# Thraix/VoxelRayTracer

Hardware: AMD Instinct MI355X
Metric: Mrays/sec + achieved HBM GB/s, 1920x1080 @ 128^3 voxels, 4 bounces (higher is better)
Workload: dtype f32

## Files before the change

### voxelraytracer_amd/csrc/vrt_cert.h

```cpp
#ifndef VRT_CERT_H
#define VRT_CERT_H

#include "vrt_walk.h"

namespace vrt {


enum : int { CERT_MISS = 0, CERT_HIT = 1, CERT_UNSURE = 2 };
constexpr int kCertRun = 3;
constexpr float kCertMargin = 1.0f / 64.0f;
constexpr int kCertMaxIter = 1024;
constexpr float kCertMaxOrigin = 4e-3f;

struct CertResult {
  int res;
  uint32_t byte;
  int axis;
  int cx, cy, cz;
  float u;
  float eu;
  float us;
  CERT_DIAG_ONLY(int iters;)
};

__device__ __forceinline__ uint32_t cell_texel(const Ctx& c, int i, int j, int k, uint32_t obase) {
  return load_u16_at(c.vox, mad24(mad24(uint32_t(k), c.p, uint32_t(j)), c.p, uint32_t(i)), obase);
}
__device__ __forceinline__ uint32_t path_texel(const Ctx& c, int i, int j, int k, uint32_t obase) {
  const uint32_t n = uint32_t(c.n);
  if (uint32_t(i) >= n || uint32_t(j) >= n || uint32_t(k) >= n) return 0u;
  return cell_texel(c, i, j, k, obase);
}
constexpr uint32_t kTexOutside = 0x10000u;
__device__ __forceinline__ uint32_t cross_texel(const Ctx& c, int i, int j, int k, uint32_t obase) {
  const bool outside = max(max(uint32_t(i), uint32_t(j)), uint32_t(k)) >= uint32_t(c.n);
  const uint32_t idx = mad24(mad24(uint32_t(k), c.p, uint32_t(j)), c.p, uint32_t(i));
  uint32_t t = load_u16_at(c.vox, outside ? 0u : idx, obase);
  t = outside ? kTexOutside : t;
  asm volatile("" : "+v"(t));
  return t;
}
__device__ __forceinline__ bool cross_outside(uint32_t tex) { return tex >= kTexOutside; }
__device__ __forceinline__ uint32_t start_texel(const Ctx& c, int i, int j, int k, uint32_t obase) {
  const bool outside = max(max(uint32_t(i), uint32_t(j)), uint32_t(k)) >= uint32_t(c.n);
  const uint32_t idx = mad24(mad24(uint32_t(k), c.p, uint32_t(j)), c.p, uint32_t(i));
  const uint32_t t = load_u16_at(c.vox, outside ? 0u : idx, obase);
  return outside ? 0u : t;
}
__device__ __forceinline__ uint32_t alt_byte(const Ctx& c, int i, int j, int k, uint32_t obase) {
  const uint32_t n = uint32_t(c.n);
  if (uint32_t(i) > n || uint32_t(j) > n || uint32_t(k) > n) return 0u;
  return cell_texel(c, i, j, k, obase) & kVoxMask;
}
template <bool SHADOW>
__device__ __forceinline__ bool cert_event(uint32_t b, uint32_t medium) {
  return SHADOW ? (b & ~2u) != 0u : b != medium;
}

struct CertStartK {
  f3 Ps, fl1;
  int mx, my, mz;
  float b0, U2;
};
typedef const __attribute__((address_space(4))) KArgs LateKArgs;
__device__ __forceinline__ LateKArgs* late_kargs() {
  LateKArgs* ka = (LateKArgs*)__builtin_amdgcn_kernarg_segment_ptr();
  asm volatile("" : "+s"(ka));
  return ka;
}

template <bool SHADOW, bool LEAN = false, bool ED = true>
__device__ __forceinline__ CertResult cert_walk(const Ctx& c, const f3 P, const f3 D, const f3 rcp, const float U,
                                int cx, int cy, int cz, const float e0, const f3 ed,
                                const float len0b, const uint32_t medium, const uint32_t tex0 = ~0u,
                                const CertStartK* __restrict__ st0 = nullptr,
                                LateKArgs* sk = nullptr) {
  CertResult r;
  r.res = CERT_UNSURE;
  r.byte = 0u;
  r.axis = 0;
  r.cx = r.cy = r.cz = 0;
  r.u = 0.0f;
  r.eu = 0.0f;
  r.us = 0.0f;
  const bool ksun = LEAN && sk != nullptr;
  const bool kst = LEAN && st0 != nullptr;
  const int sx = ksun ? sk->sun_step[0] : (D.x > 0.0f ? 1 : -1), sy = ksun ? sk->sun_step[1] : (D.y > 0.0f ? 1 : -1),
            sz = ksun ? sk->sun_step[2] : (D.z > 0.0f ? 1 : -1);
  const int ux = ksun ? (sk->sun_step[0] > 0 ? 1 : 0) : (D.x > 0.0f ? 1 : 0), uy = ksun ? (sk->sun_step[1] > 0 ? 1 : 0) : (D.y > 0.0f ? 1 : 0),
            uz = ksun ? (sk->sun_step[2] > 0 ? 1 : 0) : (D.z > 0.0f ? 1 : 0);
  const f3 ar = mk(__builtin_fabsf(rcp.x), __builtin_fabsf(rcp.y), __builtin_fabsf(rcp.z));
  const float l1 = ksun ? sk->sun_l1 : __builtin_fabsf(D.x) + __builtin_fabsf(D.y) + __builtin_fabsf(D.z);
  const uint32_t obase =
      ksun ? sk->sun_obase : ((D.x < 0.0f ? 1u : 0u) | (D.y < 0.0f ? 2u : 0u) | (D.z < 0.0f ? 4u : 0u)) * c.ostride;
  constexpr float k24 = 2.0f * 0x1p-24f;
  const float q2 = ksun ? sk->sun_q2 : 0.5f * k24 * l1;
  const float lin = 6.0f + l1 * (len0b + 1.0f),
              con = (18.0f * 1.0000020f) * __builtin_amdgcn_rcpf(l1) + 3.0f * (len0b + 1.0f);
  const float a1 = k24 * (lin + 2.0f), b1 = ksun ? sk->sun_b1 : k24 * l1,
              b0 = kst ? st0->b0 : (ksun ? sk->walk_b0 : k24 * (3.0f * c.fn + 11.0f));
  const float c0 = k24 * (con + 2.0f * len0b) + 4e-5f + e0;
  const float g2 = ksun ? sk->sun_g2 : 2.0f * q2, g1 = 2.0f * k24 * lin, g0 = 2.0f * k24 * con + 1e-4f + e0;
  const f3 Ps = kst    ? st0->Ps
                : ksun ? mk(__uint_as_float(__float_as_uint(P.x) ^ sk->sun_neg[0]), __uint_as_float(__float_as_uint(P.y) ^ sk->sun_neg[1]),
                            __uint_as_float(__float_as_uint(P.z) ^ sk->sun_neg[2]))
                       : mk(ux ? P.x : -P.x, uy ? P.y : -P.y, uz ? P.z : -P.z);
  const f3 Da = mk(__builtin_fabsf(D.x), __builtin_fabsf(D.y), __builtin_fabsf(D.z));
  const int mx = kst ? st0->mx : ux - 1, my = kst ? st0->my : uy - 1, mz = kst ? st0->mz : uz - 1;
  f3 sig = kst ? mk((st0->fl1.x - Ps.x) * ar.x, (st0->fl1.y - Ps.y) * ar.y, (st0->fl1.z - Ps.z) * ar.z)
               : mk((float(cx + ux) - P.x) * rcp.x, (float(cy + uy) - P.y) * rcp.y, (float(cz + uz) - P.z) * rcp.z);
  uint32_t tex = (tex0 != ~0u ? tex0
                              : (LEAN ? start_texel(c, cx + sx, cy + sy, cz + sz, obase)
                                      : path_texel(c, cx + sx, cy + sy, cz + sz, obase))) +
                 (1u << kDistShift);
  CTRACE(c, 100 + int(SHADOW), cx, cy, cz, P.x, P.y, P.z, U);
  CTRACE(c, 101, D.x, D.y, D.z, e0, ed.x, ed.y, ed.z);
  CERT_DIAG_ONLY(r.iters = 0;)
  if (LEAN && PHASE_STOP(SHADOW ? 4 : 2)) {
    r.u = ((sig.x + sig.y) + (sig.z + q2)) + ((a1 + b1) + (b0 + c0)) + ((g2 + g1) + (g0 + Ps.x)) +
          ((Ps.y + Ps.z) + (Da.x + Da.y)) + ((Da.z + ar.x) + (ar.y + ar.z)) + U;
    r.cx = int(tex + obase) + mx + my + mz;
    return r;
  }
  int st = CERT_UNSURE;
  for (int guard = 0; guard < kCertMaxIter; ++guard) {
    CERT_DIAG_ONLY(r.iters = guard + 1;)
    const float s1 = __builtin_fminf(sig.x, __builtin_fminf(sig.y, sig.z));
    const float uu = gmax(s1, 0.0f);
    const float A = __builtin_fmaf(__builtin_fmaf(q2, uu, a1), uu, c0);
    const float B = __builtin_fmaf(b1, uu, b0);
    auto gam_of = [&](float arb, float edb) {
      const float g = __builtin_fmaf(B, arb, A);
      return ED ? g + edb : g;
    };
    const uint32_t G = tex >> kDistShift;
    bool jumped = false;
    if (SHADOW || medium == 0u) {
      const float fg1 = float(G) - (1.0f + kCertMargin);
      const float fb = fg1 - B;
      const float jx = __builtin_fmaf(fb, ar.x, sig.x), jy = __builtin_fmaf(fb, ar.y, sig.y),
                  jz = __builtin_fmaf(fb, ar.z, sig.z);
      const float jm = ED ? __builtin_fminf(jx - ed.x, __builtin_fminf(jy - ed.y, jz - ed.z))
                          : __builtin_fminf(jx, __builtin_fminf(jy, jz));
      const float uj = __builtin_fminf(jm - A, kst ? st0->U2 : U + 2.0f);
      CTRACE(c, 102, G, s1, uj, gam_of(ar.x, ed.x), gam_of(ar.y, ed.y), gam_of(ar.z, ed.z), 0);
      if (uj > s1) {
        const float fx = __builtin_floorf(__builtin_fmaf(uj, Da.x, Ps.x)),
                    fy = __builtin_floorf(__builtin_fmaf(uj, Da.y, Ps.y)),
                    fz = __builtin_floorf(__builtin_fmaf(uj, Da.z, Ps.z));
        cx = int(fx) ^ mx;
        cy = int(fy) ^ my;
        cz = int(fz) ^ mz;
        if constexpr (LEAN)
          sig = mk(((fx + 1.0f) - Ps.x) * ar.x, ((fy + 1.0f) - Ps.y) * ar.y, ((fz + 1.0f) - Ps.z) * ar.z);
        else
          sig = mk((float(cx + ux) - P.x) * rcp.x, (float(cy + uy) - P.y) * rcp.y, (float(cz + uz) - P.z) * rcp.z);
        tex = LEAN ? cell_texel(c, cx, cy, cz, obase) : path_texel(c, cx, cy, cz, obase);
        jumped = true;
      }
    }
    st = kCertRun;
    if (!jumped) {
      const int a = sig.x == s1 ? 0 : (sig.y == s1 ? 1 : 2);
      const f3 gam = mk(gam_of(ar.x, ed.x), gam_of(ar.y, ed.y), gam_of(ar.z, ed.z));
      const f3 back = mk(sig.x - ar.x, sig.y - ar.y, sig.z - ar.z);
      const float mback = gmax(back.x, gmax(back.y, back.z));
      const float prev = gmax(mback, 0.0f);
      const float gL = __builtin_fmaf(__builtin_fmaf(g2, uu, g1), uu, g0);
      const bool lenstop = prev > U + gL;
      const int nx = cx + (a == 0 ? sx : 0), ny = cy + (a == 1 ? sy : 0), nz = cz + (a == 2 ? sz : 0);
      const uint32_t ntex = LEAN ? cross_texel(c, nx, ny, nz, obase) : path_texel(c, nx, ny, nz, obase);
      const float ga = a == 0 ? gam.x : (a == 1 ? gam.y : gam.z);
      const float tg = ga + gmax(gam.x, gmax(gam.y, gam.z));
      if (!lenstop) r.us = prev - tg - 1e-3f;
      const bool near = __builtin_amdgcn_fmed3f(sig.x, sig.y, sig.z) - s1 < tg || s1 - mback < tg;
      const uint32_t nb = ntex & kVoxMask;
      const int na = a == 0 ? nx : (a == 1 ? ny : nz);
      const bool ev = cert_event<SHADOW>(nb, medium);
      const bool lenok = prev + gL < U;
      const bool outside = LEAN ? cross_outside(ntex) : uint32_t(na) >= uint32_t(c.n);
      int res = ev ? (lenok ? CERT_HIT : CERT_UNSURE) : (outside ? CERT_MISS : CERT_UNSURE);
      bool stop = ev || outside;
      CTRACE(c, 104, cx, cy, cz, sig.x, sig.y, sig.z, ga);
      if (lenstop || near) {
        if (lenstop) {
          stop = true;
          res = s1 - mback < 2.0f * gmax(gam.x, gmax(gam.y, gam.z)) ? CERT_UNSURE : CERT_MISS;
        } else {
          const bool ahx = a != 0 && sig.x - s1 < ga + gam.x, ahy = a != 1 && sig.y - s1 < ga + gam.y,
                     ahz = a != 2 && sig.z - s1 < ga + gam.z;
          const bool bhx = a != 0 && back.x > -gam.x && s1 - back.x < ga + gam.x;
          const bool bhy = a != 1 && back.y > -gam.y && s1 - back.y < ga + gam.y;
          const bool bhz = a != 2 && back.z > -gam.z && s1 - back.z < ga + gam.z;
          const uint32_t nf = uint32_t(ahx) | uint32_t(ahy) << 1 | uint32_t(ahz) << 2 | uint32_t(bhx) << 3 |
                              uint32_t(bhy) << 4 | uint32_t(bhz) << 5;
          CTRACE(c, 103, nx, ny, nz, s1, a, nf, nb);
          auto flag = [&](int bit, bool decoded) {
            if constexpr (LEAN) {
              uint32_t f = nf;
              asm volatile("" : "+v"(f));
              return ((f >> bit) & 1u) != 0u;
            } else {
              return decoded;
            }
          };
          if (nf != 0u && ev) {
            res = CERT_UNSURE;
            if (SHADOW && lenok && __builtin_popcount(nf) == 1) {
              bool ok = true;
              if (nf & 7u) {
                const int bx = (nf & 1u) ? sx : 0, by = (nf & 2u) ? sy : 0, bz = (nf & 4u) ? sz : 0;
                ok = cert_event<true>(alt_byte(c, cx + bx, cy + by, cz + bz, obase), 0u) ||
                     cert_event<true>(alt_byte(c, nx + bx, ny + by, nz + bz, obase), 0u);
              }
              if (ok) res = CERT_HIT;
            }
          } else if (nf != 0u) {
            const int nah = int(ahx) + int(ahy) + int(ahz);
            bool bad = false;
            if (__builtin_popcount(nf) >= 2) {
              for (int q = 1; q < 8 && !bad; ++q)
                bad = cert_event<SHADOW>(alt_byte(c, cx + ((q & 1) ? sx : 0), cy + ((q & 2) ? sy : 0),
                                                  cz + ((q & 4) ? sz : 0), obase), medium);
              bad = bad || (flag(3, bhx) && cert_event<SHADOW>(alt_byte(c, nx - sx, ny, nz, obase), medium)) ||
                    (flag(4, bhy) && cert_event<SHADOW>(alt_byte(c, nx, ny - sy, nz, obase), medium)) ||
                    (flag(5, bhz) && cert_event<SHADOW>(alt_byte(c, nx, ny, nz - sz, obase), medium));
            } else if (nah) {
              const int bx = flag(0, ahx) ? sx : 0, by = flag(1, ahy) ? sy : 0, bz = flag(2, ahz) ? sz : 0;
              bad = cert_event<SHADOW>(alt_byte(c, cx + bx, cy + by, cz + bz, obase), medium) ||
                    cert_event<SHADOW>(alt_byte(c, nx + bx, ny + by, nz + bz, obase), medium);
            } else {
              bad = cert_event<SHADOW>(alt_byte(c, nx - (flag(3, bhx) ? sx : 0), ny - (flag(4, bhy) ? sy : 0),
                                                nz - (flag(5, bhz) ? sz : 0), obase), medium);
            }
            if (bad) {
              stop = true;
              res = CERT_UNSURE;
            }
          }
        }
      }
      cx = nx;
      cy = ny;
      cz = nz;
      tex = ntex;
      st = stop ? res : kCertRun;
      if (!stop) {
        if constexpr (LEAN) {
          const int ma = a == 0 ? mx : (a == 1 ? my : mz);
          const float fp = float((na ^ ma) + 1);
          if (a == 0) sig.x = (fp - Ps.x) * ar.x;
          else if (a == 1) sig.y = (fp - Ps.y) * ar.y;
          else sig.z = (fp - Ps.z) * ar.z;
        } else {
          const int sa = a == 0 ? sx : (a == 1 ? sy : sz);
          const float np = float(na + (sa > 0 ? 1 : 0));
          if (a == 0) sig.x = (np - P.x) * rcp.x;
          else if (a == 1) sig.y = (np - P.y) * rcp.y;
          else sig.z = (np - P.z) * rcp.z;
        }
      }
    }
    asm volatile("" : "+v"(st));
    if (st != kCertRun) break;
    st = CERT_UNSURE;
  }
  r.res = st;
  {
    const float s1 = __builtin_fminf(sig.x, __builtin_fminf(sig.y, sig.z));
    const float uu = gmax(s1, 0.0f);
    const float A = __builtin_fmaf(__builtin_fmaf(q2, uu, a1), uu, c0);
    const float B = __builtin_fmaf(b1, uu, b0);
    const int a = sig.x == s1 ? 0 : (sig.y == s1 ? 1 : 2);
    const float g = __builtin_fmaf(B, a == 0 ? ar.x : (a == 1 ? ar.y : ar.z), A);
    r.byte = tex & kVoxMask;
    r.axis = a;
    r.cx = cx;
    r.cy = cy;
    r.cz = cz;
    r.u = s1;
    r.eu = ED ? g + (a == 0 ? ed.x : (a == 1 ? ed.y : ed.z)) : g;
  }
  return r;
}

__device__ __forceinline__ bool cert_start(const f3 X, const f3 D0, const f3 Dn, const f3 rcpn,
                                           int fa, float e, int cx, int cy, int cz, f3& ed) {
  ed = mk(2.0f * e * __builtin_fabsf(D0.x * rcpn.x), 2.0f * e * __builtin_fabsf(D0.y * rcpn.y),
          2.0f * e * __builtin_fabsf(D0.z * rcpn.z));
  const float d0a = fa == 0 ? D0.x : (fa == 1 ? D0.y : D0.z);
  const float rna = fa == 0 ? rcpn.x : (fa == 1 ? rcpn.y : rcpn.z);
  const float lead = (e * __builtin_fabsf(d0a) + 1e-5f) * __builtin_fabsf(rna);
  const float wx = (float(cx + (Dn.x > 0.0f)) - X.x) * rcpn.x;
  const float wy = (float(cy + (Dn.y > 0.0f)) - X.y) * rcpn.y;
  const float wz = (float(cz + (Dn.z > 0.0f)) - X.z) * rcpn.z;
  const f3 fr = mk(X.x - __builtin_floorf(X.x), X.y - __builtin_floorf(X.y), X.z - __builtin_floorf(X.z));
  const f3 dm = mk(e * __builtin_fabsf(D0.x) + 2e-5f, e * __builtin_fabsf(D0.y) + 2e-5f,
                   e * __builtin_fabsf(D0.z) + 2e-5f);
  const bool okx = fa == 0 || (wx >= lead + ed.x + 1e-4f && fr.x >= dm.x && 1.0f - fr.x >= dm.x);
  const bool oky = fa == 1 || (wy >= lead + ed.y + 1e-4f && fr.y >= dm.y && 1.0f - fr.y >= dm.y);
  const bool okz = fa == 2 || (wz >= lead + ed.z + 1e-4f && fr.z >= dm.z && 1.0f - fr.z >= dm.z);
  return okx && oky && okz;
}

__device__ __forceinline__ void cell_before(const CertResult& h, const f3 D, int& x, int& y, int& z) {
  x = h.cx - (h.axis == 0 ? (D.x > 0.0f ? 1 : -1) : 0);
  y = h.cy - (h.axis == 1 ? (D.y > 0.0f ? 1 : -1) : 0);
  z = h.cz - (h.axis == 2 ? (D.z > 0.0f ? 1 : -1) : 0);
}

__device__ __forceinline__ Hit cert_hit_record(const Ray& ray, const CertResult& h) {
  Hit hh;
  hh.found = true;
  hh.voxel = h.byte;
  hh.axis = h.axis;
  hh.vidx = -1;
  hh.len = ray.len + h.u;
  hh.point = mk(ray.pos.x + h.u * ray.dir.x, ray.pos.y + h.u * ray.dir.y, ray.pos.z + h.u * ray.dir.z);
  hh.normal = mk(0.0f, 0.0f, 0.0f);
  set_comp(hh.normal, h.axis, -gsign(comp(ray.dir, h.axis)));
  return hh;
}

template <bool TEX = false, bool LEAN = false, bool KAX = false>
__device__ __forceinline__ bool cert_shade_hit(const Ctx& c, const Ray& ray, const CertResult& h,
                                               const Hit& hh, f3& color, float4 col = float4(),
                                               LateKArgs* sk = nullptr) {
  const f3 S = c.sun_n;
  float lit, ns = 0.0f;
  if constexpr (KAX) {
    if (sk->sun_ok != 0u) {
      const int a = h.axis;
      f3 D = ray.dir;
      asm volatile("" : "+v"(D.x), "+v"(D.y), "+v"(D.z));
      const float sa = a == 0 ? S.x : (a == 1 ? S.y : S.z), da = a == 0 ? D.x : (a == 1 ? D.y : D.z);
      ns = da > 0.0f ? -sa : sa;
      const float px = S.x * D.x, py = S.y * D.y, pz = S.z * D.z;
      const float rd = ((a == 0 ? -px : px) + (a == 1 ? -py : py)) + (a == 2 ? -pz : pz);
      const uint32_t m = mat_id(h.byte);
      const float diffuse = mat_kd(m) * gmax(ns, 0.0f);
      const float specular = mat_ks(m, TEX) * gpow(gmax(rd, 0.0f), mat_exp(m, TEX));
      lit = kAmbient + diffuse + specular;
    } else {
      lit = lit_brightness<TEX>(hh, S, ray.dir);
    }
  } else {
    lit = lit_brightness<TEX>(hh, S, ray.dir);
  }
  float brightness = kAmbient;
  if (lit != kAmbient && !shadow_free_hit(h.byte, TEX)) {
    if constexpr (KAX) {
      if (sk->sun_ok == 0u || !(ns > 0.0f)) { CERT_DIAG(5); return false; }
    } else {
      if (!(dot3(hh.normal, S) > 0.0f) || !fast_path_ok(S)) { CERT_DIAG(5); return false; }
    }
    int ax, ay, az;
    cell_before(h, ray.dir, ax, ay, az);
    const uint32_t sob =
        KAX ? sk->sun_obase : ((S.x < 0.0f ? 1u : 0u) | (S.y < 0.0f ? 2u : 0u) | (S.z < 0.0f ? 4u : 0u)) * c.ostride;
    const uint32_t t0 = path_texel(c, ax + (KAX ? sk->sun_step[0] : (S.x > 0.0f ? 1 : -1)), ay + (KAX ? sk->sun_step[1] : (S.y > 0.0f ? 1 : -1)),
                                   az + (KAX ? sk->sun_step[2] : (S.z > 0.0f ? 1 : -1)), sob);
    f3 ed;
    if (!cert_start(hh.point, ray.dir, S, c.sun_rcp, h.axis, h.eu, ax, ay, az, ed)) {
      CERT_DIAG(6);
      return false;
    }
    const uint32_t n = uint32_t(c.n);
    if (uint32_t(ax) >= n || uint32_t(ay) >= n || uint32_t(az) >= n) { CERT_DIAG(7); return false; }
    if (cert_event<true>(cell_texel(c, ax, ay, az, sob) & kVoxMask, 0u)) { CERT_DIAG(7); return false; }
    const CertResult s = cert_walk<true, LEAN>(c, hh.point, S, c.sun_rcp, c.max_len - hh.len, ax, ay, az,
                                         h.eu, ed, hh.len, 0u, t0, nullptr, KAX ? sk : nullptr);
    if (LEAN && (PHASE_STOP(4) || PHASE_STOP(5))) {
      color = mk(s.u + float(s.res), lit + float(s.cx), 0.0f);
      return true;
    }
    if (s.res == CERT_UNSURE) { CERT_DIAG(8); return false; }
    CERT_DIAG(9);
    brightness = s.res == CERT_HIT ? kAmbient : lit;
  } else {
    CERT_DIAG(4);
  }
  if (!TEX) col = get_color<false>(c, hh);
  color.x = mixf(color.x, col.x * col.w * brightness, ray.energy);
  color.y = mixf(color.y, col.y * col.w * brightness, ray.energy);
  color.z = mixf(color.z, col.z * col.w * brightness, ray.energy);
  return true;
}

template <bool LEAN = false>
__device__ __forceinline__ CertResult cert_march(const Ctx& c, Ray& ray, int cx, int cy, int cz, float e0, f3 ed) {
  CertResult h;
  h.res = CERT_UNSURE;
  uint32_t medium = ray.voxel;
  int internal = 0;
  for (int seg = 0; seg < 32; ++seg) {
    if (!fast_path_ok(ray.dir) || !(e0 < kCertMaxOrigin)) { CERT_DIAG(24); return h; }
    const f3 rcp = mk(__builtin_amdgcn_rcpf(ray.dir.x), __builtin_amdgcn_rcpf(ray.dir.y),
                      __builtin_amdgcn_rcpf(ray.dir.z));
    h = cert_walk<false, LEAN>(c, ray.pos, ray.dir, rcp, c.max_len - ray.len, cx, cy, cz, e0, ed, ray.len,
                               medium);
    if (h.res == CERT_UNSURE) CERT_DIAG(25);
    if (h.res != CERT_HIT || h.byte != 0u) return h;
    CERT_DIAG(30);
    h.res = CERT_UNSURE;
    const Hit eh = cert_hit_record(ray, h);
    const f3 D0 = ray.dir;
    const f3 fr = mk(eh.point.x - __builtin_floorf(eh.point.x), eh.point.y - __builtin_floorf(eh.point.y),
                     eh.point.z - __builtin_floorf(eh.point.z));
    const f3 dm = mk(h.eu * __builtin_fabsf(D0.x) + 2e-5f, h.eu * __builtin_fabsf(D0.y) + 2e-5f,
                     h.eu * __builtin_fabsf(D0.z) + 2e-5f);
    if ((h.axis != 0 && !(fr.x >= dm.x && 1.0f - fr.x >= dm.x)) ||
        (h.axis != 1 && !(fr.y >= dm.y && 1.0f - fr.y >= dm.y)) ||
        (h.axis != 2 && !(fr.z >= dm.z && 1.0f - fr.z >= dm.z))) {
      CERT_DIAG(26);
      return h;
    }
    const float eta = mat_refr(get_voxel(c, eh.point + eh.normal * 0.5f)) /
                      mat_refr(get_voxel(c, eh.point - eh.normal * 0.5f));
    const f3 rd = refract3(normalize3(D0), eh.normal, eta);
    const bool tir = rd.x == 0.0f && rd.y == 0.0f && rd.z == 0.0f;
    if (tir ? !(c.refl_noise == 0.0f && zero_noise_exact(reflect3(D0, eh.normal)))
            : !(c.refr_noise == 0.0f && zero_noise_exact(rd))) {
      CERT_DIAG(27);
      return h;
    }
    Counters kk;
#pragma unroll
    for (int q = 0; q < VRT_CNT_COUNT; ++q) kk.c[q] = 0;
    Ray nr = refraction_ray<false>(c, ray, eh, kk);
    nr.tdepth--;
    if (nr.voxel == medium) {
      internal++;
      if (internal > 10) {
        nr.dir = D0;
        nr.voxel = 0u;
      }
    }
    medium = nr.voxel;
    int nx = h.cx, ny = h.cy, nz = h.cz;
    if ((comp(nr.dir, h.axis) > 0.0f) != (comp(D0, h.axis) > 0.0f)) cell_before(h, D0, nx, ny, nz);
    if (!fast_path_ok(nr.dir)) { CERT_DIAG(28); return h; }
    const f3 rcpn = mk(__builtin_amdgcn_rcpf(nr.dir.x), __builtin_amdgcn_rcpf(nr.dir.y),
                       __builtin_amdgcn_rcpf(nr.dir.z));
    f3 edn;
    if (!cert_start(eh.point, D0, nr.dir, rcpn, h.axis, h.eu, nx, ny, nz, edn)) { CERT_DIAG(28); return h; }
    ray = nr;
    const uint32_t n = uint32_t(c.n);
    if (uint32_t(nx) >= n || uint32_t(ny) >= n || uint32_t(nz) >= n) {
      h.res = CERT_MISS;
      return h;
    }
    cx = nx;
    cy = ny;
    cz = nz;
    e0 = h.eu;
    ed = edn;
  }
  CERT_DIAG(29);
  h.res = CERT_UNSURE;
  return h;
}

struct TreeRay {
  Ray ray;
  int cx, cy, cz;
  float e0;
  f3 ed;
};
constexpr int kTreeWords = 14;
template <int NL>
__device__ __forceinline__ void tree_put(float4* __restrict__ a, float* __restrict__ b, const TreeRay& t) {
  a[0] = make_float4(t.ray.pos.x, t.ray.pos.y, t.ray.pos.z, t.ray.dir.x);
  a[1] = make_float4(t.ray.dir.y, t.ray.dir.z, t.ray.len, t.ray.energy);
  a[2] = make_float4(t.e0, t.ed.x, t.ed.y, t.ed.z);
  b[0] = __uint_as_float(uint32_t(t.cx) | uint32_t(t.cy) << 10 | uint32_t(t.cz) << 20);
  b[NL] = __uint_as_float(uint32_t(t.ray.rdepth) | uint32_t(t.ray.tdepth) << 16);
}
template <int NL>
__device__ __forceinline__ TreeRay tree_get(const float4* __restrict__ a, const float* __restrict__ b) {
  TreeRay t;
  const float4 a0 = a[0], a1 = a[1], a2 = a[2];
  t.ray.pos = mk(a0.x, a0.y, a0.z);
  t.ray.dir = mk(a0.w, a1.x, a1.y);
  t.ray.len = a1.z;
  t.ray.energy = a1.w;
  t.e0 = a2.x;
  t.ed = mk(a2.y, a2.z, a2.w);
  const uint32_t w = __float_as_uint(b[0]);
  t.cx = int(w & 1023u);
  t.cy = int((w >> 10) & 1023u);
  t.cz = int((w >> 20) & 1023u);
  const uint32_t dp = __float_as_uint(b[NL]);
  t.ray.rdepth = int(dp & 0xffffu);
  t.ray.tdepth = int(dp >> 16);
  t.ray.voxel = 0u;
  return t;
}

__device__ __forceinline__ bool tree_start(const Ctx& c, const CertResult& h, const Hit& hh, const f3 d0,
                                           TreeRay& t) {
  if (!fast_path_ok(t.ray.dir)) return false;
  const uint32_t n = uint32_t(c.n);
  if (uint32_t(t.cx) >= n || uint32_t(t.cy) >= n || uint32_t(t.cz) >= n) { CERT_DIAG(31); return false; }
  const f3 rn = mk(__builtin_amdgcn_rcpf(t.ray.dir.x), __builtin_amdgcn_rcpf(t.ray.dir.y),
                   __builtin_amdgcn_rcpf(t.ray.dir.z));
  t.e0 = h.eu;
  return cert_start(hh.point, d0, t.ray.dir, rn, h.axis, h.eu, t.cx, t.cy, t.cz, t.ed);
}

template <bool TEX>
__device__ __forceinline__ bool tree_reflection(const Ctx& c, const Ray& ray, const CertResult& h, const Hit& hh,
                                                TreeRay& t) {
  if (!(c.refl_noise == 0.0f && zero_noise_exact(reflect3(ray.dir, hh.normal)))) return false;
  t.ray = reflection_ray(c, ray, hh);
  cell_before(h, ray.dir, t.cx, t.cy, t.cz);
  return tree_start(c, h, hh, ray.dir, t);
}

template <bool TEX>
__device__ __forceinline__ bool tree_refraction(const Ctx& c, const Ray& ray, const CertResult& h, const Hit& hh,
                                                TreeRay& t) {
  const float eta = mat_refr(get_voxel(c, hh.point + hh.normal * 0.5f)) /
                    mat_refr(get_voxel(c, hh.point - hh.normal * 0.5f));
  const f3 rd = refract3(normalize3(ray.dir), hh.normal, eta);
  const bool tir = rd.x == 0.0f && rd.y == 0.0f && rd.z == 0.0f;
  if (tir ? !(c.refl_noise == 0.0f && zero_noise_exact(reflect3(ray.dir, hh.normal)))
          : !(c.refr_noise == 0.0f && zero_noise_exact(rd)))
    return false;
  Counters kk;
#pragma unroll
  for (int q = 0; q < VRT_CNT_COUNT; ++q) kk.c[q] = 0;
  t.ray = refraction_ray<TEX>(c, ray, hh, kk);
  t.cx = h.cx;
  t.cy = h.cy;
  t.cz = h.cz;
  if ((comp(t.ray.dir, h.axis) > 0.0f) != (comp(ray.dir, h.axis) > 0.0f)) cell_before(h, ray.dir, t.cx, t.cy, t.cz);
  return tree_start(c, h, hh, ray.dir, t);
}

constexpr int kTreeNext = 0, kTreeDone = 1, kTreeUnsure = -1;
template <int NL, bool LEAN = false>
__device__ __forceinline__ int tree_step(const Ctx& c, int max_refl, int max_transp, Ray& ray, CertResult& h,
                                         f3& color, bool& pending, float4* __restrict__ lta,
                                         float* __restrict__ ltb) {
  Ctx lc = c;
  asm volatile("" : "+s"(lc.sun_n.x), "+s"(lc.sun_n.y), "+s"(lc.sun_n.z), "+s"(lc.sun_rcp.x),
               "+s"(lc.sun_rcp.y), "+s"(lc.sun_rcp.z));
  bool next = false;
  TreeRay t;
  CTRACE(c, 200, h.res, h.byte, h.axis, h.u, h.eu, ray.rdepth, ray.tdepth);
  CTRACE(c, 201, ray.pos.x, ray.pos.y, ray.pos.z, ray.dir.x, ray.dir.y, ray.dir.z, ray.len);
  CTRACE(c, 202, color.x, color.y, color.z, ray.energy, h.cx, h.cy, h.cz);
  if (h.res == CERT_MISS) {
    apply_sky_color(c, ray, color);
  } else {
    const Hit hh = cert_hit_record(ray, h);
    if (!cert_shade_hit<false, LEAN>(lc, ray, h, hh, color)) { CERT_DIAG(22); return kTreeUnsure; }
    const uint32_t m = mat_id(h.byte);
    const bool pr = mat_reflective(m) && ray.rdepth < max_refl;
    const bool pt = mat_transparent(m) && ray.tdepth < max_transp && get_color<false>(c, hh).w != 1.0f;
    if (pr && pt) {
      if (pending) { CERT_DIAG(18); return kTreeUnsure; }
      TreeRay r;
      if (!tree_reflection<false>(c, ray, h, hh, r)) { CERT_DIAG(19); return kTreeUnsure; }
      tree_put<NL>(lta, ltb, r);
      pending = true;
      if (!tree_refraction<false>(c, ray, h, hh, t)) { CERT_DIAG(20); return kTreeUnsure; }
      next = true;
    } else if (pr) {
      if (!tree_reflection<false>(c, ray, h, hh, t)) { CERT_DIAG(19); return kTreeUnsure; }
      next = true;
    } else if (pt) {
      if (!tree_refraction<false>(c, ray, h, hh, t)) { CERT_DIAG(20); return kTreeUnsure; }
      next = true;
    }
  }
  if (!next) {
    if (!pending) { CERT_DIAG(17); return kTreeDone; }
    pending = false;
    t = tree_get<NL>(lta, ltb);
  }
  ray = t.ray;
  h = cert_march<LEAN>(c, ray, t.cx, t.cy, t.cz, t.e0, t.ed);
  if (h.res == CERT_UNSURE) { CERT_DIAG(21); return kTreeUnsure; }
  CERT_DIAG(23);
  return kTreeNext;
}

template <int NL, bool LEAN = false>
__device__ __forceinline__ bool cert_tree(const Ctx& c, int max_refl, int max_transp, const Ray& ray0,
                                          const CertResult& h0, f3& color_out, float4* __restrict__ lta,
                                          float* __restrict__ ltb) {
  f3 color = mk(0.0f, 0.0f, 0.0f);
  Ray ray = ray0;
  CertResult h = h0;
  bool pending = false;
  CERT_DIAG(16);
  for (;;) {
    const int r = tree_step<NL, LEAN>(c, max_refl, max_transp, ray, h, color, pending, lta, ltb);
    if (r == kTreeUnsure) return false;
    if (r == kTreeDone) break;
  }
  color_out = color;
  return true;
}

__device__ __forceinline__ bool exact_start_cell(const Ctx& c, const f3 P, const f3 D, int& cx, int& cy,
                                                 int& cz) {
  const int sx = D.x > 0.0f ? 1 : -1, sy = D.y > 0.0f ? 1 : -1, sz = D.z > 0.0f ? 1 : -1;
  cx = sx > 0 ? int(__builtin_floorf(P.x)) : int(__builtin_ceilf(P.x)) - 1;
  cy = sy > 0 ? int(__builtin_floorf(P.y)) : int(__builtin_ceilf(P.y)) - 1;
  cz = sz > 0 ? int(__builtin_floorf(P.z)) : int(__builtin_ceilf(P.z)) - 1;
  const float wpx = sx > 0 ? __builtin_floorf(P.x + 1.0f) : __builtin_ceilf(P.x - 1.0f);
  const float wpy = sy > 0 ? __builtin_floorf(P.y + 1.0f) : __builtin_ceilf(P.y - 1.0f);
  const float wpz = sz > 0 ? __builtin_floorf(P.z + 1.0f) : __builtin_ceilf(P.z - 1.0f);
  const uint32_t n = uint32_t(c.n);
  if (uint32_t(cx) >= n || uint32_t(cy) >= n || uint32_t(cz) >= n) return false;
  return wpx == float(cx + (sx > 0)) && wpy == float(cy + (sy > 0)) && wpz == float(cz + (sz > 0));
}

template <bool SHADOW>
__device__ __forceinline__ bool start_layers_clear(const Ctx& c, const f3 P, const f3 D, int cx, int cy,
                                                   int cz, uint32_t medium) {
  const float p[3] = {P.x, P.y, P.z}, d[3] = {D.x, D.y, D.z};
  const int cell[3] = {cx, cy, cz};
#pragma unroll
  for (int a = 0; a < 3; ++a) {
    if (!(d[a] < 0.0f) || p[a] != __builtin_floorf(p[a])) continue;
    const float off = (0x1p-22f * __builtin_fmaxf(__builtin_fabsf(p[a]), 1.0f) + 1e-5f) / __builtin_fabsf(d[a]);
    if (off >= 1.0f) return false;
    int q[3] = {cell[0], cell[1], cell[2]};
    q[a] += 1;
    bool early[3] = {false, false, false};
#pragma unroll
    for (int b = 0; b < 3; ++b) {
      if (b == a) continue;
      const float plane = float(cell[b] + (d[b] > 0.0f ? 1 : 0));
      early[b] = (plane - p[b]) / d[b] < off;
    }
    const int b1 = a == 0 ? 1 : 0, b2 = a == 2 ? 1 : 2;
    const int s1 = d[b1] > 0.0f ? 1 : -1, s2 = d[b2] > 0.0f ? 1 : -1;
    if (SHADOW && (early[b1] || early[b2])) return false;
    int r[3];
    if (early[b1]) {
      r[0] = q[0]; r[1] = q[1]; r[2] = q[2]; r[b1] += s1;
      if (cert_event<SHADOW>(alt_byte(c, r[0], r[1], r[2], 0u), medium)) return false;
    }
    if (early[b2]) {
      r[0] = q[0]; r[1] = q[1]; r[2] = q[2]; r[b2] += s2;
      if (cert_event<SHADOW>(alt_byte(c, r[0], r[1], r[2], 0u), medium)) return false;
    }
    if (early[b1] && early[b2]) {
      r[0] = q[0]; r[1] = q[1]; r[2] = q[2]; r[b1] += s1; r[b2] += s2;
      if (cert_event<SHADOW>(alt_byte(c, r[0], r[1], r[2], 0u), medium)) return false;
    }
  }
  return true;
}

__device__ __forceinline__ int cert_shadow_exact(const Ctx& c, const Hit& h) {
  const f3 S = c.sun_n;
  int cx, cy, cz;
  if (!fast_path_ok(S) || !exact_start_cell(c, h.point, S, cx, cy, cz)) return -1;
  if (!start_layers_clear<true>(c, h.point, S, cx, cy, cz, 0u)) return -1;
  const CertResult s = cert_walk<true, false, false>(c, h.point, S, c.sun_rcp, c.max_len - h.len, cx, cy, cz,
                                                     0.0f, mk(0.0f, 0.0f, 0.0f), h.len, 0u);
  return s.res == CERT_UNSURE ? -1 : (s.res == CERT_HIT ? 1 : 0);
}

__device__ __forceinline__ bool cert_air_segment(const Ctx& c, const Ray& ray, int cx, int cy, int cz,
                                                 const f3 ed, f3& color) {
  const f3 D = ray.dir;
  const f3 rcp = mk(__builtin_amdgcn_rcpf(D.x), __builtin_amdgcn_rcpf(D.y), __builtin_amdgcn_rcpf(D.z));
  const CertResult h = cert_walk<false>(c, ray.pos, D, rcp, c.max_len - ray.len, cx, cy, cz, 0.0f, ed,
                                        ray.len, 0u);
  if (h.res == CERT_UNSURE) return false;
  if (h.res == CERT_MISS) {
    apply_sky_color(c, ray, color);
    return true;
  }
  if (mat_id(h.byte) == 2u) return false;
  return cert_shade_hit(c, ray, h, cert_hit_record(ray, h), color);
}

__device__ __forceinline__ bool cert_secondary(const Ctx& c, const Ray& ray, f3& color) {
  int cx, cy, cz;
  if (ray.voxel != 0u || !fast_path_ok(ray.dir) || !exact_start_cell(c, ray.pos, ray.dir, cx, cy, cz) ||
      !start_layers_clear<false>(c, ray.pos, ray.dir, cx, cy, cz, 0u))
    return false;
  return cert_air_segment(c, ray, cx, cy, cz, mk(0.0f, 0.0f, 0.0f), color);
}

__device__ __forceinline__ bool cert_continuation(const Ctx& c, const Ray& ray, const WalkState& w, int fa,
                                                  f3& color) {
  const f3 D = ray.dir, P = ray.pos;
  if (!fast_path_ok(D) || w.it + 3u * uint32_t(c.n) + 16u > uint32_t(VRT_MAX_STEPS)) return false;
  int cx, cy, cz;
  const float pa = comp(P, fa), da = comp(D, fa);
  const float k = __builtin_rintf(pa);
  const float sa = da > 0.0f ? 1.0f : -1.0f;
  const float delta = __builtin_fabsf((pa + sa) - (k + sa));
  if (!(delta < 1e-3f)) return false;
  {
    const int sx = D.x > 0.0f ? 1 : -1, sy = D.y > 0.0f ? 1 : -1, sz = D.z > 0.0f ? 1 : -1;
    cx = sx > 0 ? int(__builtin_floorf(P.x)) : int(__builtin_ceilf(P.x)) - 1;
    cy = sy > 0 ? int(__builtin_floorf(P.y)) : int(__builtin_ceilf(P.y)) - 1;
    cz = sz > 0 ? int(__builtin_floorf(P.z)) : int(__builtin_ceilf(P.z)) - 1;
    const float wpx = sx > 0 ? __builtin_floorf(P.x + 1.0f) : __builtin_ceilf(P.x - 1.0f);
    const float wpy = sy > 0 ? __builtin_floorf(P.y + 1.0f) : __builtin_ceilf(P.y - 1.0f);
    const float wpz = sz > 0 ? __builtin_floorf(P.z + 1.0f) : __builtin_ceilf(P.z - 1.0f);
    if ((fa != 0 && wpx != float(cx + (sx > 0))) || (fa != 1 && wpy != float(cy + (sy > 0))) ||
        (fa != 2 && wpz != float(cz + (sz > 0))))
      return false;
    if ((fa != 0 && D.x < 0.0f && P.x == __builtin_floorf(P.x)) || (fa != 1 && D.y < 0.0f && P.y == __builtin_floorf(P.y)) ||
        (fa != 2 && D.z < 0.0f && P.z == __builtin_floorf(P.z)))
      return false;
    const int ka = int(k) - (da > 0.0f ? 0 : 1);
    if (fa == 0) cx = ka;
    else if (fa == 1) cy = ka;
    else cz = ka;
  }
  const uint32_t n = uint32_t(c.n);
  if (uint32_t(cx) >= n || uint32_t(cy) >= n || uint32_t(cz) >= n) return false;
  {
    const float before = __builtin_fmaxf((k - pa) * sa, 0.0f);
    const float off = (before + 0x1p-22f * __builtin_fmaxf(__builtin_fabsf(pa), 1.0f) + 1e-5f) *
                      __builtin_fabsf(__builtin_amdgcn_rcpf(da)) * 1.00002f;
    const float tx = fa == 0 ? off : (float(cx + (D.x > 0.0f ? 1 : 0)) - P.x) * __builtin_amdgcn_rcpf(D.x);
    const float ty = fa == 1 ? off : (float(cy + (D.y > 0.0f ? 1 : 0)) - P.y) * __builtin_amdgcn_rcpf(D.y);
    const float tz = fa == 2 ? off : (float(cz + (D.z > 0.0f ? 1 : 0)) - P.z) * __builtin_amdgcn_rcpf(D.z);
    if (__builtin_fminf(tx, __builtin_fminf(ty, tz)) < off) return false;
  }
  f3 ed = mk(0.0f, 0.0f, 0.0f);
  set_comp(ed, fa, 2.0f * delta * __builtin_fabsf(__builtin_amdgcn_rcpf(da)) + 1e-6f);
  return cert_air_segment(c, ray, cx, cy, cz, ed, color);
}

__device__ __forceinline__ Hit march_cert(const Ctx& c, Ray& ray, f3& color, bool& settled, Counters& k,
                          uint32_t& steps, uint32_t& flags) {
  Hit h;
  h.found = false;
  h.vidx = -1;
  h.len = 0.0f;
  h.voxel = 0;
  h.point = mk(0.0f, 0.0f, 0.0f);
  h.normal = h.point;
  h.axis = 0;
  settled = cert_secondary(c, ray, color);
  if (settled) return h;
  WalkState w;
  walk_init(w, ray);
  uint32_t medium = ray.voxel;
  int internal = 0;
  for (;;) {
    int axis;
    int32_t vidx;
    uint32_t v;
    const int r = walk_ray<false>(c, ray.pos, ray.dir, ray.len, medium, w, axis, vidx, v);
    if (r != WALK_EVENT) break;
    f3 normal = mk(0.0f, 0.0f, 0.0f);
    set_comp(normal, axis, -gsign(comp(ray.dir, axis)));
    if (v != 0u) {
      h.found = true;
      h.voxel = v;
      h.vidx = vidx;
      h.point = w.cur;
      h.len = w.len;
      h.normal = normal;
      h.axis = axis;
      break;
    }
    Hit e;
    e.found = true;
    e.voxel = 0;
    e.vidx = vidx;
    e.point = w.cur;
    e.len = w.len;
    e.normal = normal;
    e.axis = axis;
    const f3 old_dir = ray.dir;
    ray = refraction_ray<false>(c, ray, e, k);
    ray.tdepth--;
    if (ray.voxel == medium) {
      internal++;
      if (internal > 10) {
        ray.dir = old_dir;
        ray.voxel = 0;
      }
    }
    medium = ray.voxel;
    w.t = initial_t(ray.dir, w.cur, ray.pos);
    const f3 step = sign3(ray.dir);
    const float q = ((comp(w.cur, axis) + comp(step, axis)) - comp(ray.pos, axis)) /
                        comp(ray.dir, axis) - (w.len - ray.len);
    set_comp(w.t, axis, q);
    if (medium == 0u && cert_continuation(c, ray, w, axis, color)) {
      settled = true;
      return h;
    }
  }
  return h;
}

__device__ __forceinline__ bool texel_pair(const Ctx& c, float p, float d, uint32_t slot, bool flip, uint32_t& t) {
  const float lo = p - d, hi = p + d;
  if (__builtin_floorf(lo) != __builtin_floorf(hi)) return false;
  auto idx = [&](float q) {
    const float f = q - floorf(q);
    if (!flip) {
      const float u = ((f + float(slot)) * c.atlas_fts) / c.atlas_fs;
      return cvt_flr(u * c.atlas_fs) & c.atlas_mask;
    }
    const float ty = (((1.0f - f) + float(slot)) * c.atlas_fts) / c.atlas_fs;
    return cvt_flr((1.0f - ty) * c.atlas_fs) & c.atlas_mask;
  };
  t = idx(lo);
  return t == idx(hi);
}

__device__ __forceinline__ bool cert_texel(const Ctx& c, const Ray& ray, const CertResult& h, const Hit& hh,
                                           float4& col) {
  const uint32_t m = mat_id(h.byte);
  const float px = hh.axis == 0 ? hh.point.z : hh.point.x;
  const float py = hh.axis == 2 ? hh.point.y : (hh.axis == 1 ? hh.point.z : hh.point.y);
  const float dx = hh.axis == 0 ? ray.dir.z : ray.dir.x;
  const float dy = hh.axis == 2 ? ray.dir.y : (hh.axis == 1 ? ray.dir.z : ray.dir.y);
  const float px0 = hh.axis == 0 ? ray.pos.z : ray.pos.x;
  const float py0 = hh.axis == 2 ? ray.pos.y : (hh.axis == 1 ? ray.pos.z : ray.pos.y);
  const float ex = h.eu * __builtin_fabsf(dx) +
                   0x1p-21f * (__builtin_fabsf(px0) + __builtin_fabsf(h.u * dx) + __builtin_fabsf(px) + 1.0f);
  const float ey = h.eu * __builtin_fabsf(dy) +
                   0x1p-21f * (__builtin_fabsf(py0) + __builtin_fabsf(h.u * dy) + __builtin_fabsf(py) + 1.0f);
  uint32_t i, j;
  if (!texel_pair(c, px, ex, mat_tex_x(m), false, i) || !texel_pair(c, py, ey, mat_tex_y(m), true, j)) return false;
  const uint32_t t = c.atlas[j * (c.atlas_mask + 1u) + i];
  col = make_float4(float(t & 0xFFu) / 255.0f, float((t >> 8) & 0xFFu) / 255.0f,
                    float((t >> 16) & 0xFFu) / 255.0f, float(t >> 24) / 255.0f);
  return true;
}

__device__ __forceinline__ void late_ctx(Ctx& c) {
  LateKArgs* ka = late_kargs();
  c.sky_sy = ka->sky_sy;
  c.sun_n = mk(ka->sun_n[0], ka->sun_n[1], ka->sun_n[2]);
  c.sun_rcp = mk(ka->sun_rcp[0], ka->sun_rcp[1], ka->sun_rcp[2]);
  c.atlas = ka->atlas;
  c.atlas_mask = uint32_t(ka->atlas_size) - 1u;
  c.atlas_fs = float(ka->atlas_size);
  c.atlas_fts = float(ka->atlas_tex_size);
}
template <bool TEX = false, bool TREE = false, int NL = kWgThreads, bool LEAN = false>
__device__ __forceinline__ bool cert_pixel(const Ctx& c0, const Ray& ray0, f3& color_out, int max_refl = 0,
                                           int max_transp = 0, float* __restrict__ ltb = nullptr,
                                           float* us_out = nullptr, const KArgs* ak = nullptr) {
  const f3 P = ray0.pos, D = ray0.dir;
  int cx, cy, cz;
  CertStartK st;
  if constexpr (LEAN) {
    const bool ux = D.x > 0.0f, uy = D.y > 0.0f, uz = D.z > 0.0f;
    st.Ps = mk(ux ? P.x : -P.x, uy ? P.y : -P.y, uz ? P.z : -P.z);
    st.mx = ux ? 0 : -1;
    st.my = uy ? 0 : -1;
    st.mz = uz ? 0 : -1;
    st.b0 = ak->walk_b0;
    st.U2 = ak->max_len2;
    bool ok;
    if ((ak->setup & kSetupCell) != 0u) {
      st.fl1 = mk(ux ? ak->start_fl1[0] : ak->start_fl1[3], uy ? ak->start_fl1[1] : ak->start_fl1[4],
                  uz ? ak->start_fl1[2] : ak->start_fl1[5]);
      cx = ak->start_cell[0];
      cy = ak->start_cell[1];
      cz = ak->start_cell[2];
      ok = fast_path_ok(D);
    } else {
      const f3 fl = mk(__builtin_floorf(st.Ps.x), __builtin_floorf(st.Ps.y), __builtin_floorf(st.Ps.z));
      st.fl1 = mk(fl.x + 1.0f, fl.y + 1.0f, fl.z + 1.0f);
      cx = int(fl.x) ^ st.mx;
      cy = int(fl.y) ^ st.my;
      cz = int(fl.z) ^ st.mz;
      ok = int(fast_path_ok(D)) & int(max(max(uint32_t(cx), uint32_t(cy)), uint32_t(cz)) < uint32_t(c0.n)) &
           int(__builtin_floorf(st.Ps.x + 1.0f) == st.fl1.x) & int(__builtin_floorf(st.Ps.y + 1.0f) == st.fl1.y) &
           int(__builtin_floorf(st.Ps.z + 1.0f) == st.fl1.z);
      const bool on_plane = (int(!ux) & int(fl.x == st.Ps.x)) | (int(!uy) & int(fl.y == st.Ps.y)) |
                            (int(!uz) & int(fl.z == st.Ps.z));
      if (ok & on_plane) ok = start_layers_clear<false>(c0, P, D, cx, cy, cz, 0u);
    }
    if (!ok) { CERT_DIAG(0); return false; }
  } else {
    if (!fast_path_ok(D)) { CERT_DIAG(0); return false; }
    if (!exact_start_cell(c0, P, D, cx, cy, cz) || !start_layers_clear<false>(c0, P, D, cx, cy, cz, 0u)) {
      CERT_DIAG(0);
      return false;
    }
  }
  const f3 rcp = mk(__builtin_amdgcn_rcpf(D.x), __builtin_amdgcn_rcpf(D.y), __builtin_amdgcn_rcpf(D.z));
  CertResult h = cert_walk<false, LEAN, false>(c0, P, D, rcp, c0.max_len - ray0.len, cx, cy, cz, 0.0f,
                                               mk(0.0f, 0.0f, 0.0f), 0.0f, 0u, ~0u, LEAN ? &st : nullptr);
  if (us_out) *us_out = h.us;
  CERT_DIAG_ONLY(cert_diag_iters(10, h.iters);)
  if (LEAN && (PHASE_STOP(2) || PHASE_STOP(3))) {
    color_out = mk(h.u, h.eu, float(h.cx + h.cy + h.cz + h.axis + int(h.byte) + h.res));
    return true;
  }
  if (h.res == CERT_UNSURE) { CERT_DIAG(1); return false; }
  Ctx c = c0;
  if constexpr (LEAN) late_ctx(c);
  f3 color = mk(0.0f, 0.0f, 0.0f);
  if (h.res == CERT_MISS) {
    CERT_DIAG(2);
    if (!(LEAN && PHASE_STOP(6))) apply_sky_color(c, ray0, color);
    color_out = color;
    return true;
  }
  if (mat_id(h.byte) == 2u) {
    CERT_DIAG(3);
    if constexpr (TREE && !TEX) return cert_tree<NL, LEAN>(c, max_refl, max_transp, ray0, h, color_out, c.ax, ltb);
    return false;
  }
  const Hit hh = cert_hit_record(ray0, h);
  float4 col = float4();
  if (TEX && !cert_texel(c, ray0, h, hh, col)) return false;
  if constexpr (LEAN) {
    if (!cert_shade_hit<TEX, true, true>(c, ray0, h, hh, color, col, late_kargs())) return false;
  } else {
    if (!cert_shade_hit<TEX, false>(c, ray0, h, hh, color, col)) return false;
  }
  color_out = color;
  return true;
}

}

#endif
```

Baseline: 112,700.

## Specialize certified-pass primary shading with sun launch constants and skip redundant setup

Adds a KSUN template path to the shadow walk so the sun ray's step signs come from kernel arguments at compile time. The starting sigma is computed once in a new cert_start_sun and passed in, instead of being recomputed in the walk. For the lean primary pass, the hit record skips building the normal and ray.len, the start-cell air check is skipped when the cell differs from the known start cell, and the final colour mix is replaced by a direct assignment, which assumes energy is 1 and the colour starts at zero. The intent is to cut ALU work and one voxel fetch per shadow ray, at the cost of more template specialization and reliance on these primary-ray assumptions.

After: 118,100 (median of 6 runs). +4.8%, better.

```diff
diff --git a/voxelraytracer_amd/csrc/vrt_cert.h b/voxelraytracer_amd/csrc/vrt_cert.h
--- a/voxelraytracer_amd/csrc/vrt_cert.h
+++ b/voxelraytracer_amd/csrc/vrt_cert.h
@@ -62,6 +62,9 @@
   int mx, my, mz;
   float b0, U2;
 };
+struct CertShadowK {
+  f3 sig;
+};
 typedef const __attribute__((address_space(4))) KArgs LateKArgs;
 __device__ __forceinline__ LateKArgs* late_kargs() {
   LateKArgs* ka = (LateKArgs*)__builtin_amdgcn_kernarg_segment_ptr();
@@ -69,12 +72,13 @@
   return ka;
 }
 
-template <bool SHADOW, bool LEAN = false, bool ED = true>
+template <bool SHADOW, bool LEAN = false, bool ED = true, bool KSUN = false>
 __device__ __forceinline__ CertResult cert_walk(const Ctx& c, const f3 P, const f3 D, const f3 rcp, const float U,
                                 int cx, int cy, int cz, const float e0, const f3 ed,
                                 const float len0b, const uint32_t medium, const uint32_t tex0 = ~0u,
                                 const CertStartK* __restrict__ st0 = nullptr,
-                                LateKArgs* sk = nullptr) {
+                                LateKArgs* sk = nullptr, const CertShadowK* __restrict__ sh0 = nullptr) {
+  static_assert(!KSUN || (LEAN && SHADOW), "the sun's launch constants: the certified pass's shadow walks");
   CertResult r;
   r.res = CERT_UNSURE;
   r.byte = 0u;
@@ -83,8 +87,9 @@
   r.u = 0.0f;
   r.eu = 0.0f;
   r.us = 0.0f;
-  const bool ksun = LEAN && sk != nullptr;
+  constexpr bool ksun = KSUN;
   const bool kst = LEAN && st0 != nullptr;
+  const bool ksh = KSUN && sh0 != nullptr;
   const int sx = ksun ? sk->sun_step[0] : (D.x > 0.0f ? 1 : -1), sy = ksun ? sk->sun_step[1] : (D.y > 0.0f ? 1 : -1),
             sz = ksun ? sk->sun_step[2] : (D.z > 0.0f ? 1 : -1);
   const int ux = ksun ? (sk->sun_step[0] > 0 ? 1 : 0) : (D.x > 0.0f ? 1 : 0), uy = ksun ? (sk->sun_step[1] > 0 ? 1 : 0) : (D.y > 0.0f ? 1 : 0),
@@ -107,8 +112,9 @@
                        : mk(ux ? P.x : -P.x, uy ? P.y : -P.y, uz ? P.z : -P.z);
   const f3 Da = mk(__builtin_fabsf(D.x), __builtin_fabsf(D.y), __builtin_fabsf(D.z));
   const int mx = kst ? st0->mx : ux - 1, my = kst ? st0->my : uy - 1, mz = kst ? st0->mz : uz - 1;
-  f3 sig = kst ? mk((st0->fl1.x - Ps.x) * ar.x, (st0->fl1.y - Ps.y) * ar.y, (st0->fl1.z - Ps.z) * ar.z)
-               : mk((float(cx + ux) - P.x) * rcp.x, (float(cy + uy) - P.y) * rcp.y, (float(cz + uz) - P.z) * rcp.z);
+  f3 sig = kst   ? mk((st0->fl1.x - Ps.x) * ar.x, (st0->fl1.y - Ps.y) * ar.y, (st0->fl1.z - Ps.z) * ar.z)
+           : ksh ? sh0->sig
+                 : mk((float(cx + ux) - P.x) * rcp.x, (float(cy + uy) - P.y) * rcp.y, (float(cz + uz) - P.z) * rcp.z);
   uint32_t tex = (tex0 != ~0u ? tex0
                               : (LEAN ? start_texel(c, cx + sx, cy + sy, cz + sz, obase)
                                       : path_texel(c, cx + sx, cy + sy, cz + sz, obase))) +
@@ -303,6 +309,23 @@
   return okx && oky && okz;
 }
 
+__device__ __forceinline__ bool cert_start_sun(const f3 X, const f3 D0, const float d0a, LateKArgs* sk, const f3 rcpn,
+                                               int fa, float e, int cx, int cy, int cz, f3& ed, CertShadowK& sh) {
+  ed = mk(2.0f * e * __builtin_fabsf(D0.x * rcpn.x), 2.0f * e * __builtin_fabsf(D0.y * rcpn.y),
+          2.0f * e * __builtin_fabsf(D0.z * rcpn.z));
+  const float rna = fa == 0 ? rcpn.x : (fa == 1 ? rcpn.y : rcpn.z);
+  const float lead = (e * __builtin_fabsf(d0a) + 1e-5f) * __builtin_fabsf(rna);
+  const int ux = sk->sun_step[0] > 0 ? 1 : 0, uy = sk->sun_step[1] > 0 ? 1 : 0, uz = sk->sun_step[2] > 0 ? 1 : 0;
+  sh.sig = mk((float(cx + ux) - X.x) * rcpn.x, (float(cy + uy) - X.y) * rcpn.y, (float(cz + uz) - X.z) * rcpn.z);
+  const f3 fr = mk(X.x - __builtin_floorf(X.x), X.y - __builtin_floorf(X.y), X.z - __builtin_floorf(X.z));
+  const f3 dm = mk(e * __builtin_fabsf(D0.x) + 2e-5f, e * __builtin_fabsf(D0.y) + 2e-5f,
+                   e * __builtin_fabsf(D0.z) + 2e-5f);
+  const int okx = int(fa == 0) | (int(sh.sig.x >= lead + ed.x + 1e-4f) & int(fr.x >= dm.x) & int(1.0f - fr.x >= dm.x));
+  const int oky = int(fa == 1) | (int(sh.sig.y >= lead + ed.y + 1e-4f) & int(fr.y >= dm.y) & int(1.0f - fr.y >= dm.y));
+  const int okz = int(fa == 2) | (int(sh.sig.z >= lead + ed.z + 1e-4f) & int(fr.z >= dm.z) & int(1.0f - fr.z >= dm.z));
+  return (okx & oky & okz) != 0;
+}
+
 __device__ __forceinline__ void cell_before(const CertResult& h, const f3 D, int& x, int& y, int& z) {
   x = h.cx - (h.axis == 0 ? (D.x > 0.0f ? 1 : -1) : 0);
   y = h.cy - (h.axis == 1 ? (D.y > 0.0f ? 1 : -1) : 0);
@@ -322,18 +345,48 @@
   return hh;
 }
 
+__device__ __forceinline__ f3 cert_hit_normal(const f3 D, int axis) {
+  f3 n = mk(0.0f, 0.0f, 0.0f);
+  set_comp(n, axis, -gsign(comp(D, axis)));
+  return n;
+}
+__device__ __forceinline__ Hit cert_hit_record_primary(const Ray& ray, const CertResult& h) {
+  Hit hh;
+  hh.found = true;
+  hh.voxel = h.byte;
+  hh.axis = h.axis;
+  hh.vidx = -1;
+  hh.len = h.u;
+  hh.point = mk(ray.pos.x + h.u * ray.dir.x, ray.pos.y + h.u * ray.dir.y, ray.pos.z + h.u * ray.dir.z);
+  hh.normal = mk(0.0f, 0.0f, 0.0f);
+  return hh;
+}
+
 template <bool TEX = false, bool LEAN = false, bool KAX = false>
 __device__ __forceinline__ bool cert_shade_hit(const Ctx& c, const Ray& ray, const CertResult& h,
                                                const Hit& hh, f3& color, float4 col = float4(),
                                                LateKArgs* sk = nullptr) {
   const f3 S = c.sun_n;
-  float lit, ns = 0.0f;
+  if constexpr (KAX) __builtin_assume(h.byte != 0u && h.byte != 2u);
+  float lit, ns = 0.0f, da = 0.0f;
+  auto lit_generic = [&]() {
+    if constexpr (KAX) {
+      int ga = h.axis;
+      asm volatile("" : "+v"(ga));
+      Hit hg = hh;
+      hg.normal = cert_hit_normal(ray.dir, ga);
+      return lit_brightness<TEX>(hg, S, ray.dir);
+    } else {
+      return lit_brightness<TEX>(hh, S, ray.dir);
+    }
+  };
   if constexpr (KAX) {
     if (sk->sun_ok != 0u) {
       const int a = h.axis;
       f3 D = ray.dir;
       asm volatile("" : "+v"(D.x), "+v"(D.y), "+v"(D.z));
-      const float sa = a == 0 ? S.x : (a == 1 ? S.y : S.z), da = a == 0 ? D.x : (a == 1 ? D.y : D.z);
+      const float sa = a == 0 ? S.x : (a == 1 ? S.y : S.z);
+      da = a == 0 ? D.x : (a == 1 ? D.y : D.z);
       ns = da > 0.0f ? -sa : sa;
       const float px = S.x * D.x, py = S.y * D.y, pz = S.z * D.z;
       const float rd = ((a == 0 ? -px : px) + (a == 1 ? -py : py)) + (a == 2 ? -pz : pz);
@@ -342,10 +395,10 @@
       const float specular = mat_ks(m, TEX) * gpow(gmax(rd, 0.0f), mat_exp(m, TEX));
       lit = kAmbient + diffuse + specular;
     } else {
-      lit = lit_brightness<TEX>(hh, S, ray.dir);
+      lit = lit_generic();
     }
   } else {
-    lit = lit_brightness<TEX>(hh, S, ray.dir);
+    lit = lit_generic();
   }
   float brightness = kAmbient;
   if (lit != kAmbient && !shadow_free_hit(h.byte, TEX)) {
@@ -358,18 +411,49 @@
     cell_before(h, ray.dir, ax, ay, az);
     const uint32_t sob =
         KAX ? sk->sun_obase : ((S.x < 0.0f ? 1u : 0u) | (S.y < 0.0f ? 2u : 0u) | (S.z < 0.0f ? 4u : 0u)) * c.ostride;
-    const uint32_t t0 = path_texel(c, ax + (KAX ? sk->sun_step[0] : (S.x > 0.0f ? 1 : -1)), ay + (KAX ? sk->sun_step[1] : (S.y > 0.0f ? 1 : -1)),
-                                   az + (KAX ? sk->sun_step[2] : (S.z > 0.0f ? 1 : -1)), sob);
+    const int tx = ax + (KAX ? sk->sun_step[0] : (S.x > 0.0f ? 1 : -1)), ty = ay + (KAX ? sk->sun_step[1] : (S.y > 0.0f ? 1 : -1)),
+              tz = az + (KAX ? sk->sun_step[2] : (S.z > 0.0f ? 1 : -1));
+    const uint32_t t0 = KAX ? start_texel(c, tx, ty, tz, sob) : path_texel(c, tx, ty, tz, sob);
+    if (KAX && PHASE_STOP(7)) {
+      color = mk(lit + hh.len, hh.point.x + hh.point.y + hh.point.z + da, float(int(t0) + ax + ay + az));
+      return true;
+    }
     f3 ed;
-    if (!cert_start(hh.point, ray.dir, S, c.sun_rcp, h.axis, h.eu, ax, ay, az, ed)) {
-      CERT_DIAG(6);
-      return false;
-    }
-    const uint32_t n = uint32_t(c.n);
-    if (uint32_t(ax) >= n || uint32_t(ay) >= n || uint32_t(az) >= n) { CERT_DIAG(7); return false; }
-    if (cert_event<true>(cell_texel(c, ax, ay, az, sob) & kVoxMask, 0u)) { CERT_DIAG(7); return false; }
-    const CertResult s = cert_walk<true, LEAN>(c, hh.point, S, c.sun_rcp, c.max_len - hh.len, ax, ay, az,
-                                         h.eu, ed, hh.len, 0u, t0, nullptr, KAX ? sk : nullptr);
+    CertShadowK sh;
+    bool go = true;
+    if constexpr (KAX) {
+      go = cert_start_sun(hh.point, ray.dir, da, sk, c.sun_rcp, h.axis, h.eu, ax, ay, az, ed, sh);
+      if (!go) CERT_DIAG(6);
+    } else {
+      if (!cert_start(hh.point, ray.dir, S, c.sun_rcp, h.axis, h.eu, ax, ay, az, ed)) {
+        CERT_DIAG(6);
+        return false;
+      }
+    }
+    if (KAX && PHASE_STOP(8)) {
+      color = mk(lit + hh.len + ed.x + ed.y + ed.z, sh.sig.x + sh.sig.y + sh.sig.z, float(int(t0) + ax + ay + az));
+      return true;
+    }
+    bool air_known = false;
+    if constexpr (KAX)
+      air_known = (sk->setup & kSetupCell) != 0u &&
+                  ((ax ^ sk->start_cell[0]) | (ay ^ sk->start_cell[1]) | (az ^ sk->start_cell[2])) != 0;
+    if constexpr (KAX) {
+      if (go && !air_known) {
+        const uint32_t n = uint32_t(c.n);
+        go = max(max(uint32_t(ax), uint32_t(ay)), uint32_t(az)) < n;
+        if (go) go = !cert_event<true>(cell_texel(c, ax, ay, az, sob) & kVoxMask, 0u);
+        if (!go) CERT_DIAG(7);
+      }
+      if (!go) return false;
+    } else {
+      const uint32_t n = uint32_t(c.n);
+      if (uint32_t(ax) >= n || uint32_t(ay) >= n || uint32_t(az) >= n) { CERT_DIAG(7); return false; }
+      if (cert_event<true>(cell_texel(c, ax, ay, az, sob) & kVoxMask, 0u)) { CERT_DIAG(7); return false; }
+    }
+    const CertResult s = cert_walk<true, LEAN, true, KAX>(c, hh.point, S, c.sun_rcp, c.max_len - hh.len, ax, ay, az,
+                                                          h.eu, ed, hh.len, 0u, t0, nullptr, KAX ? sk : nullptr,
+                                                          KAX ? &sh : nullptr);
     if (LEAN && (PHASE_STOP(4) || PHASE_STOP(5))) {
       color = mk(s.u + float(s.res), lit + float(s.cx), 0.0f);
       return true;
@@ -381,9 +465,13 @@
     CERT_DIAG(4);
   }
   if (!TEX) col = get_color<false>(c, hh);
-  color.x = mixf(color.x, col.x * col.w * brightness, ray.energy);
-  color.y = mixf(color.y, col.y * col.w * brightness, ray.energy);
-  color.z = mixf(color.z, col.z * col.w * brightness, ray.energy);
+  if constexpr (KAX) {
+    color = mk(col.x * col.w * brightness, col.y * col.w * brightness, col.z * col.w * brightness);
+  } else {
+    color.x = mixf(color.x, col.x * col.w * brightness, ray.energy);
+    color.y = mixf(color.y, col.y * col.w * brightness, ray.energy);
+    color.z = mixf(color.z, col.z * col.w * brightness, ray.energy);
+  }
   return true;
 }
 
@@ -917,7 +1005,7 @@
     if constexpr (TREE && !TEX) return cert_tree<NL, LEAN>(c, max_refl, max_transp, ray0, h, color_out, c.ax, ltb);
     return false;
   }
-  const Hit hh = cert_hit_record(ray0, h);
+  const Hit hh = LEAN ? cert_hit_record_primary(ray0, h) : cert_hit_record(ray0, h);
   float4 col = float4();
   if (TEX && !cert_texel(c, ray0, h, hh, col)) return false;
   if constexpr (LEAN) {
```
